# wangheda/youtube-8m

Measured on AMD Instinct MI355X. Metric: training videos/sec, higher is better.
Workload: dtype f32; 1 GPU; BASELINE configs[3]: LstmModel (2 x BasicLSTMCell(1024), dynamic_rnn over F=300) on raw uint8 [B,300,1152] frames + MoeModel head (2 mixtures, V=4716), fp32 training step (fwd+bwd+clip+Adam); per_gpu_batch=128, global_batch=128, frames=300, parallelism=dp1, params=113902808

## Files before the change

### include/yt8m_hip.h

```cpp
#ifndef YT8M_HIP_H
#define YT8M_HIP_H
#include <stdint.h>

#ifdef __cplusplus
extern "C" {
#endif

typedef void* yt8m_stream_t;

enum yt8m_status { YT8M_OK = 0, YT8M_E_BADARG = -1, YT8M_E_SHAPE = -2, YT8M_E_HIP = -3, YT8M_E_RCCL = -4 };
enum yt8m_label_dtype { YT8M_LABEL_U8 = 0, YT8M_LABEL_F32 = 1 };

int yt8m_abi_version(void);
const char* yt8m_last_error(void);
const char* yt8m_built_arch(void);

int yt8m_prof_enable(int on);
int yt8m_prof_reset(void);
int yt8m_prof_get(int family, int64_t* launches, double* total_ms);
int yt8m_prof_get_flops(int family, double* flops);
int yt8m_prof_get_bytes(int family, double* bytes);

int yt8m_probe_mfma_f32(int iters, int blocks, float* sink, yt8m_stream_t stream);
int yt8m_probe_mfma_bf16(int iters, int blocks, int random_operands, float* sink, yt8m_stream_t stream);
int yt8m_probe_copy_f32(const float* src, float* dst, int64_t n, yt8m_stream_t stream);
int yt8m_probe_placement(int* out, int blocks, int spin_ticks, yt8m_stream_t stream);
int yt8m_stream_create_cu_mask(const uint32_t* mask, int words, yt8m_stream_t* stream);
int yt8m_stream_destroy(yt8m_stream_t stream);

int yt8m_gemm_f32(int transA, int transB, int64_t M, int64_t N, int64_t K,
                  const float* A, int64_t lda, const float* B, int64_t ldb,
                  float* C, int64_t ldc, const float* bias, float beta, yt8m_stream_t stream);

int yt8m_gemm_f32_batched(int transA, int transB, int64_t M, int64_t N, int64_t K,
                          const float* A, int64_t lda, int64_t strideA, const float* B, int64_t ldb, int64_t strideB,
                          float* C, int64_t ldc, int64_t strideC, float beta, int64_t batch, yt8m_stream_t stream);

typedef struct yt8m_gemm_problem {
  int64_t M, N, K;
  const void* A; int64_t lda;
  const void* B; int64_t ldb;
  float* C; int64_t ldc;
  const float* bias;
  float beta;
} yt8m_gemm_problem;
int64_t yt8m_gemm_workspace_bytes(void);
int yt8m_gemm_f32_grouped(int transA, int transB, int nprob, const yt8m_gemm_problem* probs, void* workspace,
                          int64_t workspace_bytes, yt8m_stream_t stream);
int yt8m_gemm_bf16_nt_grouped(int nprob, const yt8m_gemm_problem* probs, void* workspace, int64_t workspace_bytes,
                              yt8m_stream_t stream);
int64_t yt8m_x3_image_bytes(int64_t rows, int64_t K);
int yt8m_x3_split(const float* src, int64_t R, int64_t C, int64_t ld, float scale, void* plain, void* trans, yt8m_stream_t stream);
int yt8m_gemm_x3_nt_grouped(int nprob, const yt8m_gemm_problem* probs, void* workspace, int64_t workspace_bytes,
                            yt8m_stream_t stream);
int yt8m_h2_split(const float* src, int64_t R, int64_t C, int64_t ld, float scale, const float* dscale, void* plain, void* trans,
                  float* colpart, yt8m_stream_t stream);
int yt8m_h2_absmax(const float* src, int64_t R, int64_t C, int64_t ld, void* word, yt8m_stream_t stream);
int yt8m_h2_degraded(uint64_t* counts, int reset, yt8m_stream_t stream);
int yt8m_h2_split_dropout(const float* src, int64_t R, int64_t C, float scale, const float* dscale, void* plain, void* trans,
                          float keep_prob, uint64_t seed, int64_t offset, yt8m_stream_t stream);
int yt8m_h2_split_rowmax(const float* src, int64_t R, int64_t C, int64_t ld, const void* rowmax, float* inv, void* plain,
                         yt8m_stream_t stream);
int yt8m_h2_split_ex(const float* src, int64_t R, int64_t C, int64_t ld, float scale, const void* dscale, const float* rowscale, void* plain,
                     void* trans, void* trans_scaled, float* colpart, float* colpart_scaled, yt8m_stream_t stream);
int yt8m_gemm_h1x2_nt_ex(int64_t M, int64_t N, int64_t K, const void* A1, int64_t ska, const void* B2, int64_t skb, float* C, int64_t ldc,
                         const float* bias, float alpha, const void* dsb, const float* rowscale, const float* colsum, float colsum_scale,
                         float beta, void* workspace, int64_t workspace_bytes, yt8m_stream_t stream);
int yt8m_h2_rowscales(const float* src, int64_t R, int64_t C, int64_t ld, float* S, float* inv, yt8m_stream_t stream);
int yt8m_h2_split_rows(const float* src, int64_t R, int64_t C, int64_t ld, const float* S, void* plain, yt8m_stream_t stream);
int yt8m_gemm_h2_nt_ex(int64_t M, int64_t N, int64_t K, const void* A2, int64_t ska, const void* B2, int64_t skb, float* C, int64_t ldc,
                       const float* bias, float alpha, const void* dsa, const void* dsb, const float* rowscale, float beta, void* workspace,
                       int64_t workspace_bytes, yt8m_stream_t stream);
int yt8m_timepool_max_f32(const float* y, int64_t F, int64_t B, int64_t N, int64_t ldy, float* out, int32_t* idx, int64_t ldo,
                          yt8m_stream_t stream);
int yt8m_timepool_shiftmax_f32(const float* z, int64_t F, int64_t B, int64_t ldz, int nfilt, const int32_t* fs, const int32_t* ncol, float* out,
                               int32_t* idx, int64_t ldo, yt8m_stream_t stream);
int yt8m_u8_cnn_pool_dw(const uint8_t* q, const float* r_tm, const int32_t* idx, const float* g, int64_t ldg, int64_t B, int64_t F, int64_t D,
                        int64_t N, int64_t fs, float* dW, float beta, yt8m_stream_t stream);
int yt8m_f32_cnn_pool_dw(const float* x, int64_t ldx, const int32_t* idx, const float* g, int64_t ldg, int64_t B, int64_t F, int64_t D,
                         int64_t N, int64_t fs, float* dW, int64_t lddw, float beta, yt8m_stream_t stream);
int yt8m_f32_cnn_pool_dx(const int32_t* idx, const float* g, int64_t ldg, int64_t B, int64_t F, int64_t D, int nfilt, const float* const* wt,
                         const int32_t* fs, const int32_t* ncol, float* dx, int64_t lddx, yt8m_stream_t stream);
int yt8m_u8_frames_image_f16(const uint8_t* q, const int32_t* num_frames, int64_t B, int64_t F, int64_t D, float eps, void* image,
                             float* x_tm, float* r_out, yt8m_stream_t stream);
int yt8m_u8_frames_image_t_f16(const uint8_t* q, const int32_t* num_frames, int64_t B, int64_t F, int64_t D, void* image_t,
                               yt8m_stream_t stream);
int yt8m_gemm_h2_nt_grouped(int nprob, const yt8m_gemm_problem* probs, const float* alphas, const float* const* dsa,
                            const float* const* dsb, void* workspace, int64_t workspace_bytes, yt8m_stream_t stream);
int yt8m_x3_set_combine(int mode);
int yt8m_x3_set_schedule(int mode);
#define YT8M_GEMM_ROLE_DW 0x100
#define YT8M_GEMM_ROLE_H2 0x200
int yt8m_gemm_x3_pays(int64_t M, int64_t N, int64_t K);
int64_t yt8m_gemm_auto_scratch_bytes(int transA, int transB, int nprob, const yt8m_gemm_problem* probs);
int yt8m_gemm_auto_grouped(int transA, int transB, int nprob, const yt8m_gemm_problem* probs, void* workspace,
                           int64_t workspace_bytes, void* image_scratch, int64_t image_scratch_bytes, uint64_t* used_x3,
                           yt8m_stream_t stream);
int yt8m_gemm_auto_grouped_ex(int transA, int transB, int nprob, const yt8m_gemm_problem* probs, const float* const* absmaxA,
                              const float* const* absmaxB, void* workspace, int64_t workspace_bytes, void* image_scratch,
                              int64_t image_scratch_bytes, uint64_t* used_x3, yt8m_stream_t stream);
int yt8m_gemm_x1x3_nt(int64_t M, int64_t N, int64_t K, const void* A1, const void* B3, float* C, int64_t ldc, const float* bias,
                      const float* rowscale, const float* colsum, float colsum_scale, void* workspace, int64_t workspace_bytes,
                      yt8m_stream_t stream);
int yt8m_gemm_x1x3_nt_ex(int64_t M, int64_t N, int64_t K, const void* A1, int64_t ska, const void* B3, int64_t skb, float* C,
                         int64_t ldc, const float* bias, float alpha, const float* rowscale, const float* colsum,
                         float colsum_scale, float beta, void* workspace, int64_t workspace_bytes, yt8m_stream_t stream);
int yt8m_bf16_image(const float* src, int64_t R, int64_t C, int64_t ld, float scale, void* plain, void* trans, yt8m_stream_t stream);
int yt8m_gemm_b1_nt_grouped(int nprob, const yt8m_gemm_problem* probs, void* workspace, int64_t workspace_bytes, yt8m_stream_t stream);
int yt8m_gemm_b1_nt_grouped_bf16c(int nprob, const yt8m_gemm_problem* probs, unsigned c_bf16_mask, void* workspace, int64_t workspace_bytes,
                                  yt8m_stream_t stream);
int yt8m_moe_mix_fwd_bf16z(const void* Zg, const void* Ze, float* p, int64_t B, int64_t V, int M, yt8m_stream_t stream);
int yt8m_moe_mix_bwd_bf16_images_z16(const void* Zg, const void* Ze, const float* dp, const void* labels, int label_dtype, int64_t B,
                                     int64_t V, int M, float eps, float dscale, const float* upstream_dev, void* dZg_img, int64_t g_kb,
                                     void* dZg_t_img, int64_t gt_kb, void* dZe_img, int64_t e_kb, void* dZe_t_img, int64_t et_kb,
                                     float* be_part, yt8m_stream_t stream);
int yt8m_bf16_image_colsum(const float* src, int64_t R, int64_t C, int64_t ld, float scale, const float* rowscale, void* plain,
                           void* trans, void* trans_scaled, float* colpart, float* colpart_scaled, yt8m_stream_t stream);
int yt8m_gemm_b1_nt_ex(int64_t M, int64_t N, int64_t K, const void* A1, int64_t ska, const void* B1, int64_t skb, float* C, int64_t ldc,
                       const float* bias, float alpha, const float* rowscale, const float* colsum, float colsum_scale, float beta,
                       void* workspace, int64_t workspace_bytes, yt8m_stream_t stream);
int yt8m_x3_split_ex(const float* src, int64_t R, int64_t C, int64_t ld, float scale, const float* rowscale, void* plain,
                     void* trans, void* trans_scaled, yt8m_stream_t stream);
int yt8m_x3_split_colsum(const float* src, int64_t R, int64_t C, int64_t ld, float scale, const float* rowscale, void* plain,
                         void* trans, void* trans_scaled, float* colpart, float* colpart_scaled, yt8m_stream_t stream);
int yt8m_cast_f32_bf16(const float* src, int64_t rows, int64_t cols, int64_t ld, void* dst, int64_t dst_ld, int transpose,
                       yt8m_stream_t stream);
int yt8m_cast_f32_bf16_dual(const float* src, int64_t rows, int64_t cols, int64_t ld, void* dst_plain, int64_t plain_ld,
                            void* dst_trans, int64_t trans_ld, yt8m_stream_t stream);

int yt8m_l2norm_fwd_f32(const float* x, float* y, int64_t rows, int64_t cols, float eps, yt8m_stream_t stream);
int yt8m_l2norm_bwd_f32(const float* x, const float* dy, float* dx, int64_t rows, int64_t cols, float eps,
                        yt8m_stream_t stream);
int yt8m_dequant_l2norm_u8(const uint8_t* q, const int32_t* num_frames, float* x,
                           int64_t B, int64_t F, int64_t D, float eps, yt8m_stream_t stream);
int yt8m_dequant_mean_l2norm_u8(const uint8_t* q, const int32_t* num_frames, float* x,
                                int64_t B, int64_t F, int64_t D, float eps, yt8m_stream_t stream);
int yt8m_resolution_mean_u8(const uint8_t* q, const int32_t* num_frames, float* y, int32_t* num_frames_out, int64_t B, int64_t F,
// ... 590 lines not shown
```

### youtube-8m_amd/csrc/common.h

```cpp
#pragma once
#include <hip/hip_runtime.h>
#include <stdint.h>
#include <stdio.h>
#include <string.h>
#include "../../include/yt8m_hip.h"

namespace yt8m {

extern thread_local char g_err[512];

inline int fail(int code, const char* fmt, const char* a = "", long long b = 0, long long c = 0) {
  snprintf(g_err, sizeof(g_err), fmt, a, b, c);
  return code;
}

#define YT8M_HIP_CHECK(expr)                                                              \
  do {                                                                                    \
    hipError_t _e = (expr);                                                               \
    if (_e != hipSuccess) {                                                               \
      snprintf(yt8m::g_err, sizeof(yt8m::g_err), "%s failed: %s (%s:%d)", #expr,          \
               hipGetErrorString(_e), __FILE__, __LINE__);                                \
      return YT8M_E_HIP;                                                                  \
    }                                                                                     \
  } while (0)

#define YT8M_REQUIRE(cond, code, msg)                                                     \
  do {                                                                                    \
    if (!(cond)) {                                                                        \
      snprintf(yt8m::g_err, sizeof(yt8m::g_err), "%s: requirement failed: %s", __func__, msg); \
      return code;                                                                        \
    }                                                                                     \
  } while (0)

enum Family { F_GEMM = 0, F_MOE_FUSED = 1, F_ELEMENTWISE = 2, F_OPTIM = 3, F_LSTM = 4, F_NETVLAD = 5, F_LSTM_BWD = 6, F_GEMM_X3 = 7,
              F_GEMM_X1X3 = 8,
              F_VLAD_ROWS = 9,
              F_VLAD_COLS = 10,
              F_NETVLAD_FWD = 11,
              F_GEMM_H2 = 12,
              F_GEMM_H1X2 = 13,
              F_COUNT = 14 };

struct ProfScope {
  int fam;
  hipStream_t s;
  bool on;
  hipEvent_t e0, e1;
  double flops;
  double bytes;
  ProfScope(int family, hipStream_t stream, double algorithmic_flops = 0.0, double algorithmic_bytes = 0.0);
  ~ProfScope();
};

bool prof_enabled();

struct GraphKey {
  int kind;
  int pad;
  const void* p[10];
  int64_t v[8];
};
}
#include <atomic>
#include <functional>
namespace yt8m {
int run_chain(const GraphKey& key, hipStream_t s, const std::function<int()>& launch_all);

inline hipStream_t as_stream(yt8m_stream_t s) { return reinterpret_cast<hipStream_t>(s); }

bool gemm_bf16_big_ok(int nprob, const yt8m_gemm_problem* probs);
int gemm_bf16_big_launch(int nprob, const yt8m_gemm_problem* probs, void* workspace, int64_t workspace_bytes, hipStream_t s);

struct DeviceOnce {
  std::atomic<bool> done[64];
  DeviceOnce() { for (auto& d : done) d.store(false); }
  hipError_t lds(const void* fn, int bytes) {
    int dev = 0;
    hipError_t e = hipGetDevice(&dev);
    if (e != hipSuccess) return e;
    if (dev >= 0 && dev < 64 && done[dev].load(std::memory_order_acquire)) return hipSuccess;
    e = hipFuncSetAttribute(fn, hipFuncAttributeMaxDynamicSharedMemorySize, bytes);
    if (e == hipSuccess && dev >= 0 && dev < 64) done[dev].store(true, std::memory_order_release);
    return e;
  }
};

inline int launch_status(const char* what) {
  hipError_t e = hipGetLastError();
  if (e != hipSuccess) {
    snprintf(g_err, sizeof(g_err), "launch of %s failed: %s", what, hipGetErrorString(e));
    return YT8M_E_HIP;
  }
  return YT8M_OK;
}

}

inline bool aligned16(const void* p) { return (reinterpret_cast<uintptr_t>(p) & 15) == 0; }
inline int64_t cdiv(int64_t a, int64_t b) { return (a + b - 1) / b; }
inline int64_t up4(int64_t a) { return (a + 3) & ~(int64_t)3; }

__device__ __forceinline__ float wave_sum(float v) {
#pragma unroll
  for (int o = 32; o > 0; o >>= 1) v += __shfl_xor(v, o, 64);
  return v;
}
__device__ __forceinline__ float wave_max(float v) {
#pragma unroll
  for (int o = 32; o > 0; o >>= 1) v = fmaxf(v, __shfl_xor(v, o, 64));
  return v;
}
__device__ __forceinline__ float block_sum_256(float v, float* red ) {
  v = wave_sum(v);
  const int lane = threadIdx.x & 63, w = threadIdx.x >> 6;
  __syncthreads();
  if (lane == 0) red[w] = v;
  __syncthreads();
  return red[0] + red[1] + red[2] + red[3];
}
__device__ __forceinline__ float block_max_256(float v, float* red) {
  v = wave_max(v);
  const int lane = threadIdx.x & 63, w = threadIdx.x >> 6;
  __syncthreads();
  if (lane == 0) red[w] = v;
  __syncthreads();
  return fmaxf(fmaxf(red[0], red[1]), fmaxf(red[2], red[3]));
}
template <int N>
__device__ __forceinline__ void block_sums_256(float (&v)[N], float* red ) {
#pragma unroll
  for (int k = 0; k < N; ++k) v[k] = wave_sum(v[k]);
  const int lane = threadIdx.x & 63, w = threadIdx.x >> 6;
  __syncthreads();
  if (lane == 0) {
#pragma unroll
    for (int k = 0; k < N; ++k) red[w * N + k] = v[k];
  }
  __syncthreads();
#pragma unroll
  for (int k = 0; k < N; ++k) v[k] = red[k] + red[N + k] + red[2 * N + k] + red[3 * N + k];
}
__device__ __forceinline__ float sigmoidf_(float z) { return 1.0f / (1.0f + expf(-z)); }

__device__ __forceinline__ float fast_sigmoid(float x) {
  return __builtin_amdgcn_rcpf(1.0f + __builtin_amdgcn_exp2f(-1.4426950408889634f * x));
}
__device__ __forceinline__ float fast_tanh(float x) {
  return 1.0f - 2.0f * __builtin_amdgcn_rcpf(1.0f + __builtin_amdgcn_exp2f(2.8853900817779268f * x));
}

template <int VW>
__device__ __forceinline__ void ldv(const float* p, float (&r)[VW]) {
  if constexpr (VW == 4) {
    const float4 q = *reinterpret_cast<const float4*>(p);
// ... 22 lines not shown
```

### youtube-8m_amd/csrc/gemm_f32.hip

```cpp
#include "common.h"

#ifdef YT8M_GEMM_TIMING
__device__ unsigned long long yt8m_gemm_phase[8];
extern "C" int yt8m_debug_gemm_phase(unsigned long long* out) {
  return hipMemcpyFromSymbol(out, HIP_SYMBOL(yt8m_gemm_phase), sizeof(unsigned long long) * 8) == hipSuccess ? 0 : -3;
}
#endif

#ifndef YT8M_GEMM_TEPI
#define YT8M_GEMM_TEPI 0
#endif

namespace {

constexpr bool TEPI = YT8M_GEMM_TEPI != 0;
constexpr int BM = 128, BN = 128, BK = 16;
constexpr int TILE_FLOATS = BK * 128;
constexpr int STAGES = 3;

typedef float f32x16 __attribute__((ext_vector_type(16)));

struct GemmArgs {
  const float* A;
  const float* B;
// ... 594 lines not shown

static int grouped_launch(int transA, int transB, int bf16, int nprob, const yt8m_gemm_problem* probs, void* workspace,
                          int64_t workspace_bytes, yt8m_stream_t stream) {
  using namespace yt8m;
  YT8M_REQUIRE(nprob >= 1 && nprob <= MAX_GROUP && probs, YT8M_E_BADARG, "1..4 problems");
  GroupArgs G;
  G.nprob = 0;
  int64_t T = 0;
  for (int i = 0; i < nprob; ++i) {
    const yt8m_gemm_problem& q = probs[i];
    GemmArgs g;
    int rc;
    if (bf16) {
      YT8M_REQUIRE(q.K % 2 == 0 && q.lda % 2 == 0 && q.ldb % 2 == 0, YT8M_E_SHAPE, "bf16 GEMM needs even K / lda / ldb");
      rc = fill_problem(g, 0, 1, q.M, q.N, q.K / 2, static_cast<const float*>(q.A), q.lda / 2, static_cast<const float*>(q.B),
                        q.ldb / 2, q.C, q.ldc, q.bias, q.beta);
    } else {
      rc = fill_problem(g, transA, transB, q.M, q.N, q.K, static_cast<const float*>(q.A), q.lda, static_cast<const float*>(q.B),
                        q.ldb, q.C, q.ldc, q.bias, q.beta);
    }
    if (rc != YT8M_OK) return rc;
    if (q.M == 0 || q.N == 0) continue;
    G.p[G.nprob] = g;
    G.tile_base[G.nprob] = (int)T;
    T += (int64_t)g.tiles_m * g.tiles_n;
    ++G.nprob;
  }
  if (G.nprob == 0) return YT8M_OK;
  YT8M_REQUIRE(T < (1LL << 30), YT8M_E_SHAPE, "too many tiles");
  for (int i = G.nprob; i <= MAX_GROUP; ++i) G.tile_base[i] = (int)T;
  for (int i = G.nprob; i < MAX_GROUP; ++i) G.p[i] = G.p[0];
  G.T = (int)T;
  G.P = T < SLOTS ? (int)T : SLOTS;
  G.full_rounds = (int)(T / G.P);
  G.rem = (int)(T - (int64_t)G.full_rounds * G.P);
  G.S = 1;
  G.ws = static_cast<float*>(workspace);
  if (T < SLOTS) {
    G.P = SLOTS;
    G.full_rounds = 0;
    G.rem = (int)T;
  }
  if (G.rem > 0) {
    int min_nk = 1 << 30, max_nk = 0;
    for (int i = 0; i < G.nprob; ++i) {
      const int nk = (G.p[i].K + BK - 1) / BK;
      if (nk < min_nk) min_nk = nk;
      if (nk > max_nk) max_nk = nk;
    }
    int Smax = min_nk / 8;
    if (Smax > 96) Smax = 96;
    const int64_t ws_items = workspace ? workspace_bytes / ((int64_t)BM * BN * (int64_t)sizeof(float)) : 0;
    if ((int64_t)G.rem * Smax > ws_items) Smax = (int)(ws_items / G.rem);
    int S = 1;
    double best = 1e30;
    for (int c = 1; c <= Smax; ++c) {
      const int64_t rounds = ((int64_t)G.rem * c + G.P - 1) / G.P;
      const double cost = (double)rounds * ((double)max_nk / c + 8.0) + (c > 1 ? 2.0 : 0.0);
      if (cost < best * 0.98) { best = cost; S = c; }
    }
    G.S = S;
  }
  hipStream_t s = as_stream(stream);
  double fl = 0.0;
  for (int i = 0; i < G.nprob; ++i) fl += 2.0 * (double)G.p[i].M * (double)G.p[i].N * (double)G.p[i].K;
  ProfScope prof(F_GEMM, s, fl);
  const int64_t grid = (int64_t)G.full_rounds * G.P + (int64_t)G.rem * G.S;
  int kmax = 0;
  for (int i = 0; i < G.nprob; ++i) kmax = std::max(kmax, G.p[i].K);
  if (bf16)
    hipLaunchKernelGGL((gemm_grouped_kernel<true, true, true>), dim3((unsigned)grid), dim3(256), 0, s, G);
  else if (transA && !transB && kmax <= 2048)
    hipLaunchKernelGGL((gemm_grouped_kernel<false, false, false, true>), dim3((unsigned)grid), dim3(256), 0, s, G);
  else
    launch_by_layout<GroupArgs>(transA, transB, gemm_grouped_kernel<true, false, false>, gemm_grouped_kernel<false, false, false>,
                                gemm_grouped_kernel<true, true, false>, gemm_grouped_kernel<false, true, false>,
                                dim3((unsigned)grid), s, G);
  if (G.S > 1) hipLaunchKernelGGL(splitk_fixup_kernel, dim3((unsigned)G.rem * 16), dim3(256), 0, s, G);
  return launch_status("gemm_grouped_kernel");
}

extern "C" int yt8m_gemm_f32_grouped(int transA, int transB, int nprob, const yt8m_gemm_problem* probs, void* workspace,
                                     int64_t workspace_bytes, yt8m_stream_t stream) {
  return grouped_launch(transA, transB, 0, nprob, probs, workspace, workspace_bytes, stream);
}

extern "C" int yt8m_gemm_bf16_nt_grouped(int nprob, const yt8m_gemm_problem* probs, void* workspace, int64_t workspace_bytes,
                                         yt8m_stream_t stream) {
  using namespace yt8m;
  YT8M_REQUIRE(nprob >= 1 && nprob <= MAX_GROUP && probs, YT8M_E_BADARG, "1..4 problems");
  bool simple = true;
  for (int i = 0; i < nprob; ++i) {
    const yt8m_gemm_problem& q = probs[i];
    simple = simple && q.M >= 0 && q.N >= 0 && q.K >= 0 && q.A && q.B && q.C && q.lda >= q.K && q.ldb >= q.K && q.ldc >= q.N &&
             (q.beta == 0.f || q.beta == 1.f);
  }
  if (simple && gemm_bf16_big_ok(nprob, probs)) {
    double fl = 0.0;
    for (int i = 0; i < nprob; ++i) fl += 2.0 * (double)probs[i].M * (double)probs[i].N * (double)probs[i].K;
    ProfScope prof(F_GEMM, as_stream(stream), fl);
    return gemm_bf16_big_launch(nprob, probs, workspace, workspace_bytes, as_stream(stream));
  }
  return grouped_launch(0, 1, 1, nprob, probs, workspace, workspace_bytes, stream);
}

extern "C" int yt8m_gemm_f32(int transA, int transB, int64_t M, int64_t N, int64_t K, const float* A, int64_t lda,
                             const float* B, int64_t ldb, float* C, int64_t ldc, const float* bias, float beta,
                             yt8m_stream_t stream) {
  return gemm_launch(transA, transB, M, N, K, A, lda, 0, B, ldb, 0, C, ldc, 0, bias, beta, 1, stream);
}

extern "C" int yt8m_gemm_f32_batched(int transA, int transB, int64_t M, int64_t N, int64_t K, const float* A, int64_t lda,
                                     int64_t strideA, const float* B, int64_t ldb, int64_t strideB, float* C, int64_t ldc,
                                     int64_t strideC, float beta, int64_t batch, yt8m_stream_t stream) {
  return gemm_launch(transA, transB, M, N, K, A, lda, strideA, B, ldb, strideB, C, ldc, strideC, nullptr, beta, batch, stream);
}
```

Baseline: 8316 videos/s.

## Route small-row fp32 GEMMs with large weights to bf16x3 MFMA row kernels

Adds a specialised path for fp32 GEMMs with at most 128 rows and large weight matrices, such as the MoE logits and the matching dx GEMMs. The activations are split into a three-term bf16 image. The weights are split on the fly into LDS, and a six-product bf16 MFMA sum emulates fp32 precision. The dx path uses split-K partials plus a combine kernel. The aim is to use matrix cores on these skinny, weight-bandwidth-bound GEMMs instead of the generic fp32 tiled kernel, at the cost of extra split launches, workspace use and small numeric differences.

```diff
diff --git a/include/yt8m_hip.h b/include/yt8m_hip.h
--- a/include/yt8m_hip.h
+++ b/include/yt8m_hip.h
@@ -53,6 +53,7 @@
 int yt8m_x3_split(const float* src, int64_t R, int64_t C, int64_t ld, float scale, void* plain, void* trans, yt8m_stream_t stream);
 int yt8m_gemm_x3_nt_grouped(int nprob, const yt8m_gemm_problem* probs, void* workspace, int64_t workspace_bytes,
                             yt8m_stream_t stream);
+#define YT8M_GEMM_ROLE_ROWS 0x400
 int yt8m_h2_split(const float* src, int64_t R, int64_t C, int64_t ld, float scale, const float* dscale, void* plain, void* trans,
                   float* colpart, yt8m_stream_t stream);
 int yt8m_h2_absmax(const float* src, int64_t R, int64_t C, int64_t ld, void* word, yt8m_stream_t stream);
diff --git a/youtube-8m_amd/csrc/common.h b/youtube-8m_amd/csrc/common.h
--- a/youtube-8m_amd/csrc/common.h
+++ b/youtube-8m_amd/csrc/common.h
@@ -70,6 +70,9 @@
 
 bool gemm_bf16_big_ok(int nprob, const yt8m_gemm_problem* probs);
 int gemm_bf16_big_launch(int nprob, const yt8m_gemm_problem* probs, void* workspace, int64_t workspace_bytes, hipStream_t s);
+bool gemm_rows_route(int transA, int transB, int nprob, const yt8m_gemm_problem* probs, int64_t workspace_bytes);
+int gemm_rows_logits(int nprob, const yt8m_gemm_problem* probs, void* workspace, int64_t workspace_bytes, yt8m_stream_t stream);
+int gemm_rows_dx(int nprob, const yt8m_gemm_problem* probs, void* workspace, int64_t workspace_bytes, yt8m_stream_t stream);
 
 struct DeviceOnce {
   std::atomic<bool> done[64];
diff --git a/youtube-8m_amd/csrc/gemm_f32.hip b/youtube-8m_amd/csrc/gemm_f32.hip
--- a/youtube-8m_amd/csrc/gemm_f32.hip
+++ b/youtube-8m_amd/csrc/gemm_f32.hip
@@ -700,6 +700,17 @@
 
 extern "C" int yt8m_gemm_f32_grouped(int transA, int transB, int nprob, const yt8m_gemm_problem* probs, void* workspace,
                                      int64_t workspace_bytes, yt8m_stream_t stream) {
+  const bool declared = (transA & YT8M_GEMM_ROLE_ROWS) != 0;
+  transA &= ~YT8M_GEMM_ROLE_ROWS;
+  if (declared) YT8M_REQUIRE(transA == 0 && nprob >= 1 && nprob <= MAX_GROUP && probs, YT8M_E_BADARG, "YT8M_GEMM_ROLE_ROWS: transA = 0, 1..4 problems");
+  if (declared || yt8m::gemm_rows_route(transA, transB, nprob, probs, workspace ? workspace_bytes : 0)) {
+    if (!transB) return yt8m::gemm_rows_logits(nprob, probs, workspace, workspace_bytes, stream);
+    for (int i = 0; i < nprob; ++i) {
+      const int rc = yt8m::gemm_rows_dx(1, probs + i, workspace, workspace_bytes, stream);
+      if (rc != YT8M_OK) return rc;
+    }
+    return YT8M_OK;
+  }
   return grouped_launch(transA, transB, 0, nprob, probs, workspace, workspace_bytes, stream);
 }
 
diff --git a/youtube-8m_amd/csrc/gemm_rows.hip b/youtube-8m_amd/csrc/gemm_rows.hip
--- /dev/null
+++ b/youtube-8m_amd/csrc/gemm_rows.hip
@@ -0,0 +1,518 @@
+#include "common.h"
+#include "rows_plan.h"
+#include <stdlib.h>
+
+namespace {
+
+using namespace yt8m_rows;
+
+typedef float f32x16 __attribute__((ext_vector_type(16)));
+typedef float f32x2 __attribute__((ext_vector_type(2)));
+typedef __bf16 bf16x8 __attribute__((ext_vector_type(8)));
+typedef __bf16 bf16x2 __attribute__((ext_vector_type(2)));
+typedef short s16x4 __attribute__((ext_vector_type(4)));
+typedef short s16x8 __attribute__((ext_vector_type(8)));
+
+constexpr int IMG_BLOCK_F = 256;
+
+__device__ __forceinline__ unsigned pk_bf16(float a, float b) {
+  const f32x2 f = {a, b};
+  return __builtin_bit_cast(unsigned, __builtin_convertvector(f, bf16x2));
+}
+__device__ __forceinline__ void split3_pair(float a, float b, unsigned& h0, unsigned& h1, unsigned& h2) {
+  h0 = pk_bf16(a, b);
+  const bool fa = (__float_as_uint(a) & 0x7F800000u) != 0x7F800000u, fb = (__float_as_uint(b) & 0x7F800000u) != 0x7F800000u;
+  const float ra = fa ? a - __uint_as_float(h0 << 16) : 0.f;
+  const float rb = fb ? b - __uint_as_float(h0 & 0xFFFF0000u) : 0.f;
+  h1 = pk_bf16(ra, rb);
+  h2 = pk_bf16(ra - __uint_as_float(h1 << 16), rb - __uint_as_float(h1 & 0xFFFF0000u));
+}
+__device__ __forceinline__ void store_split4(char* at, int plane, float4 v) {
+  unsigned a0, a1, a2, b0, b1, b2;
+  split3_pair(v.x, v.y, a0, a1, a2);
+  split3_pair(v.z, v.w, b0, b1, b2);
+  *reinterpret_cast<uint2*>(at) = make_uint2(a0, b0);
+  *reinterpret_cast<uint2*>(at + plane) = make_uint2(a1, b1);
+  *reinterpret_cast<uint2*>(at + 2 * plane) = make_uint2(a2, b2);
+}
+template <bool VEC>
+__device__ __forceinline__ float4 load4(const float* __restrict__ p, int c, int ncols, int ld, bool ok) {
+  float4 v = {0.f, 0.f, 0.f, 0.f};
+  if constexpr (VEC) {
+    v = *reinterpret_cast<const float4*>(p + min(c, ld - 4));
+  } else if (ok) {
+    if (c + 0 < ncols) v.x = p[c + 0];
+    if (c + 1 < ncols) v.y = p[c + 1];
+    if (c + 2 < ncols) v.z = p[c + 2];
+    if (c + 3 < ncols) v.w = p[c + 3];
+  }
+  return v;
+}
+__device__ __forceinline__ float4 mask4(float4 t, int c, int ncols, bool ok) {
+  float4 v;
+  v.x = (ok && c + 0 < ncols) ? t.x : 0.f;
+  v.y = (ok && c + 1 < ncols) ? t.y : 0.f;
+  v.z = (ok && c + 2 < ncols) ? t.z : 0.f;
+  v.w = (ok && c + 3 < ncols) ? t.w : 0.f;
+  return v;
+}
+__device__ __forceinline__ bf16x8 load_a(const float* __restrict__ img, int rg, int kb, int KB, int p, int li, int lk) {
+  const int64_t block = (int64_t)rg * KB + min(kb, KB - 1);
+  return __builtin_bit_cast(bf16x8, *reinterpret_cast<const float4*>(img + (block * 3 + p) * IMG_BLOCK_F + li * 8 + 4 * (lk ^ ((li >> 3) & 1))));
+}
+__device__ __forceinline__ bf16x8 keep_a(bf16x8 a, bool inside) {
+  return inside ? a : __builtin_bit_cast(bf16x8, make_float4(0.f, 0.f, 0.f, 0.f));
+}
+__device__ __forceinline__ f32x16 six(const bf16x8 (&a)[3], const bf16x8 (&b)[3], f32x16 c) {
+  c = __builtin_amdgcn_mfma_f32_32x32x16_bf16(a[2], b[0], c, 0, 0, 0);
+  c = __builtin_amdgcn_mfma_f32_32x32x16_bf16(a[1], b[0], c, 0, 0, 0);
+  c = __builtin_amdgcn_mfma_f32_32x32x16_bf16(a[1], b[1], c, 0, 0, 0);
+  c = __builtin_amdgcn_mfma_f32_32x32x16_bf16(a[0], b[0], c, 0, 0, 0);
+  c = __builtin_amdgcn_mfma_f32_32x32x16_bf16(a[0], b[1], c, 0, 0, 0);
+  c = __builtin_amdgcn_mfma_f32_32x32x16_bf16(a[0], b[2], c, 0, 0, 0);
+  return c;
+}
+constexpr int FLUSH_KBLOCKS = 8;
+template <int T>
+__device__ __forceinline__ void flush(f32x16 (&run)[T], f32x16 (&total)[T]) {
+#pragma unroll
+  for (int j = 0; j < T; ++j) {
+    total[j] += run[j];
+#pragma unroll
+    for (int r = 0; r < 16; ++r) run[j][r] = 0.f;
+  }
+}
+
+struct LArgs {
+  const float* W;
+  const float* img;
+  float* C;
+  const float* bias;
+  int64_t ldw, ldc;
+  int M, N, K, accumulate;
+};
+struct LGroup {
+  LArgs p[MAX_PROBS];
+  int slab_base[MAX_PROBS + 1];
+  int nprob;
+};
+
+constexpr int L_ROW_B = LOGITS_SLAB * 2;
+constexpr int L_PLANE_B = LOGITS_KBLK * L_ROW_B;
+constexpr int L_STAGE_B = 3 * L_PLANE_B;
+constexpr int L_LDS_B = 2 * L_STAGE_B;
+constexpr int L_LOADS = LOGITS_KBLK * (LOGITS_SLAB / 4) / 512;
+static_assert(LOGITS_KBLK * (LOGITS_SLAB / 4) % 512 == 0, "a stage is a whole number of float4 per thread");
+
+template <bool VEC>
+__global__ __launch_bounds__(512) void rows_logits_kernel(const LGroup G) {
+  extern __shared__ __attribute__((aligned(16))) char lds[];
+  int q = 0;
+  while (q + 1 < G.nprob && (int)blockIdx.x >= G.slab_base[q + 1]) ++q;
+  const LArgs& g = G.p[q];
+  const int n0 = ((int)blockIdx.x - G.slab_base[q]) * LOGITS_SLAB;
+  const int tid = threadIdx.x, lane = tid & 63, wave = tid >> 6;
+  const int li = lane & 31, lk = lane >> 5;
+  const int mt = wave & 3, kg = wave >> 2;
+  const int mtiles = (g.M + 31) >> 5;
+  const bool active = mt < mtiles;
+  const int rg = min(mt, mtiles - 1);
+  const int KB = (g.K + 15) >> 4;
+  const int nblk = (g.K + LOGITS_KBLK - 1) / LOGITS_KBLK;
+
+  int lrow[L_LOADS], lc4[L_LOADS];
+#pragma unroll
+  for (int i = 0; i < L_LOADS; ++i) {
+    const int idx = tid + 512 * i;
+    lrow[i] = idx / (LOGITS_SLAB / 4);
+    lc4[i] = idx % (LOGITS_SLAB / 4);
+  }
+  auto load_w = [&](int blk, float4 (&v)[L_LOADS]) __attribute__((always_inline)) {
+#pragma unroll
+    for (int i = 0; i < L_LOADS; ++i) {
+      const int k = blk * LOGITS_KBLK + lrow[i];
+      v[i] = load4<VEC>(g.W + (int64_t)min(k, g.K - 1) * g.ldw, n0 + lc4[i] * 4, g.N, (int)g.ldw, k < g.K);
+    }
+  };
+  auto store_w = [&](int blk, const float4 (&v)[L_LOADS]) __attribute__((always_inline)) {
+#pragma unroll
+    for (int i = 0; i < L_LOADS; ++i)
+      store_split4(lds + (blk & 1) * L_STAGE_B + lrow[i] * L_ROW_B + lc4[i] * 8, L_PLANE_B,
+                   mask4(v[i], n0 + lc4[i] * 4, g.N, blk * LOGITS_KBLK + lrow[i] < g.K));
+  };
+  auto keep_x = [&](int blk, const bf16x8 (&from)[2][3], bf16x8 (&to)[2][3]) __attribute__((always_inline)) {
+#pragma unroll
+    for (int s = 0; s < 2; ++s)
+#pragma unroll
+      for (int p = 0; p < 3; ++p) to[s][p] = keep_a(from[s][p], blk * (LOGITS_KBLK / 16) + 2 * kg + s < KB);
+  };
+  auto load_x = [&](int blk, bf16x8 (&a)[2][3]) __attribute__((always_inline)) {
+#pragma unroll
+    for (int s = 0; s < 2; ++s) {
+      const int kb = blk * (LOGITS_KBLK / 16) + 2 * kg + s;
+#pragma unroll
+      for (int p = 0; p < 3; ++p) a[s][p] = load_a(g.img, rg, kb, KB, p, li, lk);
+    }
+  };
+  const int tq = (lane >> 2) & 3, tp = lane & 3, gq = lane >> 4;
+  const int tr_off = (8 * (gq >> 1) + tq) * L_ROW_B + (16 * (gq & 1) + 4 * tp) * 2;
+
+  f32x16 acc[3], run[3];
+#pragma unroll
+  for (int j = 0; j < 3; ++j)
+#pragma unroll
+    for (int r = 0; r < 16; ++r) acc[j][r] = run[j][r] = 0.f;
+
+  float4 wv[L_LOADS];
+  bf16x8 xa[2][3], xn[2][3];
+  load_w(0, wv);
+  load_x(0, xn);
+  store_w(0, wv);
+  keep_x(0, xn, xa);
+  __syncthreads();
+  for (int blk = 0; blk < nblk; ++blk) {
+    const bool more = blk + 1 < nblk;
+    const int nxt = more ? blk + 1 : blk;
+    load_w(nxt, wv);
+    load_x(nxt, xn);
+    __builtin_amdgcn_sched_barrier(0);
+    {
+      const char* S = lds + (blk & 1) * L_STAGE_B + tr_off;
+#pragma unroll
+      for (int s = 0; s < 2; ++s) {
+        const char* Sk = S + (2 * kg + s) * 16 * L_ROW_B;
+#pragma unroll
+        for (int j = 0; j < 3; ++j) {
+          bf16x8 b[3];
+#pragma unroll
+          for (int p = 0; p < 3; ++p) {
+            const char* at = Sk + p * L_PLANE_B + j * 64;
+            const s16x4 lo = __builtin_amdgcn_ds_read_tr16_b64_v4i16((__attribute__((address_space(3))) s16x4*)(at));
+            const s16x4 hi = __builtin_amdgcn_ds_read_tr16_b64_v4i16((__attribute__((address_space(3))) s16x4*)(at + 4 * L_ROW_B));
+            const s16x8 both = {lo[0], lo[1], lo[2], lo[3], hi[0], hi[1], hi[2], hi[3]};
+            b[p] = __builtin_bit_cast(bf16x8, both);
+          }
+          run[j] = six(xa[s], b, run[j]);
+        }
+      }
+    }
+    if ((blk + 1) % (FLUSH_KBLOCKS / 2) == 0) flush(run, acc);
+    __builtin_amdgcn_sched_barrier(0);
+    if (more) {
+      store_w(blk + 1, wv);
+      keep_x(blk + 1, xn, xa);
+    }
+    __syncthreads();
+  }
+  flush(run, acc);
+  float* X = reinterpret_cast<float*>(lds) + (mt * 3 * 16) * 64 + lane;
+  if (kg == 1) {
+#pragma unroll
+    for (int j = 0; j < 3; ++j)
+#pragma unroll
+      for (int r = 0; r < 16; ++r) X[(j * 16 + r) * 64] = acc[j][r];
+  }
+  __syncthreads();
+  if (kg == 1 || !active) return;
+#pragma unroll
+  for (int j = 0; j < 3; ++j) {
+    const int col = n0 + 32 * j + li;
+    if (col >= g.N) continue;
+    const float bv = g.bias ? g.bias[col] : 0.f;
+#pragma unroll
+    for (int r = 0; r < 16; ++r) {
+      const int row = mt * 32 + (r & 3) + 8 * (r >> 2) + 4 * lk;
+      if (row < g.M) {
+        float* c = g.C + (int64_t)row * g.ldc + col;
+        float v = acc[j][r] + X[(j * 16 + r) * 64] + bv;
+        if (g.accumulate) v += *c;
+        *c = v;
+      }
+    }
+  }
+}
+
+struct DArgs {
+  const float* W[MAX_PROBS];
+  const float* img[MAX_PROBS];
+  int64_t ldw[MAX_PROBS];
+  int N[MAX_PROBS];
+  int split_prob[DX_MAX_SPLITS], split_g0[DX_MAX_SPLITS], split_g1[DX_MAX_SPLITS];
+  float* part;
+  float* C;
+  int64_t ldc;
+  int M, Kout, S, accumulate;
+};
+
+constexpr int D_ROW_B = DX_GROUP * 2 + 16;
+constexpr int D_PLANE_B = DX_SLAB * D_ROW_B;
+constexpr int D_STAGE_B = 3 * D_PLANE_B;
+constexpr int D_LDS_B = 2 * D_STAGE_B;
+constexpr int D_LOADS = DX_SLAB * (DX_GROUP / 4) / 512;
+
+template <bool VEC>
+__global__ __launch_bounds__(512) void rows_dx_kernel(const DArgs g) {
+  extern __shared__ __attribute__((aligned(16))) char lds[];
+  const int split = (int)blockIdx.x % g.S, slab = (int)blockIdx.x / g.S;
+  const int q = g.split_prob[split], g0 = g.split_g0[split], g1 = g.split_g1[split];
+  const int tid = threadIdx.x, lane = tid & 63, wave = tid >> 6;
+  const int li = lane & 31, lk = lane >> 5;
+  const int mt = wave & 3, cp = wave >> 2;
+  const int mtiles = (g.M + 31) >> 5;
+  const bool active = mt < mtiles;
+  const int rg = min(mt, mtiles - 1);
+  const int N = g.N[q];
+  const int KB = (N + 15) >> 4;
+  const int64_t ldw = g.ldw[q];
+  const int o0 = slab * DX_SLAB;
+  const float* W = g.W[q];
+  const float* img = g.img[q];
+
+  int lrow[D_LOADS], lc4[D_LOADS];
+#pragma unroll
+  for (int i = 0; i < D_LOADS; ++i) {
+    const int idx = tid + 512 * i;
+    lrow[i] = idx / (DX_GROUP / 4);
+    lc4[i] = idx % (DX_GROUP / 4);
+  }
+  auto load_w = [&](int grp, float4 (&v)[D_LOADS]) __attribute__((always_inline)) {
+#pragma unroll
+    for (int i = 0; i < D_LOADS; ++i) {
+      const int row = o0 + lrow[i];
+      v[i] = load4<VEC>(W + (int64_t)min(row, g.Kout - 1) * ldw, grp * DX_GROUP + lc4[i] * 4, N, (int)ldw, row < g.Kout);
+    }
+  };
+  auto store_w = [&](int grp, const float4 (&v)[D_LOADS]) __attribute__((always_inline)) {
+#pragma unroll
+    for (int i = 0; i < D_LOADS; ++i)
+      store_split4(lds + ((grp - g0) & 1) * D_STAGE_B + lrow[i] * D_ROW_B + lc4[i] * 8, D_PLANE_B,
+                   mask4(v[i], grp * DX_GROUP + lc4[i] * 4, N, o0 + lrow[i] < g.Kout));
+  };
+  auto keep_z = [&](int grp, const bf16x8 (&from)[4][3], bf16x8 (&to)[4][3]) __attribute__((always_inline)) {
+#pragma unroll
+    for (int s = 0; s < 4; ++s)
+#pragma unroll
+      for (int p = 0; p < 3; ++p) to[s][p] = keep_a(from[s][p], grp * (DX_GROUP / 16) + s < KB);
+  };
+  auto load_z = [&](int grp, int s, bf16x8 (&a)[3]) __attribute__((always_inline)) {
+    const int kb = grp * (DX_GROUP / 16) + s;
+#pragma unroll
+    for (int p = 0; p < 3; ++p) a[p] = load_a(img, rg, kb, KB, p, li, lk);
+  };
+
+  f32x16 acc[2], run[2];
+#pragma unroll
+  for (int j = 0; j < 2; ++j)
+#pragma unroll
+    for (int r = 0; r < 16; ++r) acc[j][r] = run[j][r] = 0.f;
+
+  float4 wv[D_LOADS];
+  bf16x8 za[4][3], zn[4][3];
+  load_w(g0, wv);
+#pragma unroll
+  for (int s = 0; s < 4; ++s) load_z(g0, s, zn[s]);
+  store_w(g0, wv);
+  keep_z(g0, zn, za);
+  __syncthreads();
+  for (int grp = g0; grp < g1; ++grp) {
+    const int st = (grp - g0) & 1;
+    const bool more = grp + 1 < g1;
+    const int nxt = more ? grp + 1 : grp;
+    load_w(nxt, wv);
+#pragma unroll
+    for (int s = 0; s < 4; ++s) load_z(nxt, s, zn[s]);
+    __builtin_amdgcn_sched_barrier(0);
+    {
+      const char* S = lds + st * D_STAGE_B + (64 * cp + li) * D_ROW_B + lk * 16;
+#pragma unroll
+      for (int s = 0; s < 4; ++s) {
+#pragma unroll
+        for (int j = 0; j < 2; ++j) {
+          bf16x8 b[3];
+#pragma unroll
+          for (int p = 0; p < 3; ++p)
+            b[p] = __builtin_bit_cast(bf16x8, *reinterpret_cast<const float4*>(S + p * D_PLANE_B + j * 32 * D_ROW_B + s * 32));
+          run[j] = six(za[s], b, run[j]);
+        }
+      }
+    }
+    if ((grp - g0 + 1) % (FLUSH_KBLOCKS / 4) == 0) flush(run, acc);
+    __builtin_amdgcn_sched_barrier(0);
+    if (more) {
+      store_w(grp + 1, wv);
+      keep_z(grp + 1, zn, za);
+    }
+    __syncthreads();
+  }
+  flush(run, acc);
+  if (!active) return;
+  float* P = g.part + ((int64_t)slab * g.S + split) * (MAX_ROWS * DX_SLAB);
+#pragma unroll
+  for (int j = 0; j < 2; ++j)
+#pragma unroll
+    for (int r = 0; r < 16; ++r) {
+      const int row = mt * 32 + (r & 3) + 8 * (r >> 2) + 4 * lk;
+      P[row * DX_SLAB + 64 * cp + 32 * j + li] = acc[j][r];
+    }
+}
+
+__global__ __launch_bounds__(256) void rows_dx_combine_kernel(const float* __restrict__ part, float* __restrict__ C, int64_t ldc, int M,
+                                                              int Kout, int S, int accumulate) {
+  const int o4 = (Kout + 3) >> 2;
+  const int64_t idx = (int64_t)blockIdx.x * 256 + threadIdx.x;
+  if (idx >= (int64_t)M * o4) return;
+  const int m = (int)(idx / o4), o = (int)(idx % o4) * 4;
+  const int slab = o / DX_SLAB, c = o % DX_SLAB;
+  const float* p = part + (int64_t)slab * S * (MAX_ROWS * DX_SLAB) + m * DX_SLAB + c;
+  float4 v = *reinterpret_cast<const float4*>(p);
+  for (int s = 1; s < S; ++s) {
+    const float4 t = *reinterpret_cast<const float4*>(p + (int64_t)s * (MAX_ROWS * DX_SLAB));
+    v.x += t.x; v.y += t.y; v.z += t.z; v.w += t.w;
+  }
+  float* c4 = C + (int64_t)m * ldc + o;
+  if (o + 3 < Kout && (ldc & 3) == 0 && (reinterpret_cast<uintptr_t>(C) & 15) == 0) {
+    if (accumulate) {
+      const float4 old = *reinterpret_cast<const float4*>(c4);
+      v.x += old.x; v.y += old.y; v.z += old.z; v.w += old.w;
+    }
+    *reinterpret_cast<float4*>(c4) = v;
+  } else {
+    const float vv[4] = {v.x, v.y, v.z, v.w};
+    for (int e = 0; e < 4 && o + e < Kout; ++e) c4[e] = accumulate ? vv[e] + c4[e] : vv[e];
+  }
+}
+
+}
+
+using namespace yt8m;
+
+static bool rows_enabled() {
+  static const bool off = getenv("YT8M_GEMM_ROWS") != nullptr && atoi(getenv("YT8M_GEMM_ROWS")) == 0;
+  return !off;
+}
+
+static int64_t rows_workspace_bytes(bool dx, int nprob, const yt8m_gemm_problem* probs) {
+  int64_t M[MAX_PROBS], N[MAX_PROBS], K[MAX_PROBS];
+  int same[MAX_PROBS];
+  for (int i = 0; i < nprob; ++i) {
+    M[i] = probs[i].M; N[i] = probs[i].N; K[i] = probs[i].K;
+    same[i] = i;
+    for (int j = 0; j < i; ++j)
+      if (probs[j].A == probs[i].A && probs[j].lda == probs[i].lda && M[j] == M[i] && K[j] == K[i]) { same[i] = j; break; }
+  }
+  if (dx) return plan_dx(nprob, M[0], N[0], K).workspace_bytes;
+  return plan_logits(nprob, M, N, K, same).workspace_bytes;
+}
+
+bool yt8m::gemm_rows_route(int transA, int transB, int nprob, const yt8m_gemm_problem* probs, int64_t workspace_bytes) {
+  if (!rows_enabled() || transA != 0 || nprob < 1 || nprob > MAX_PROBS || !probs) return false;
+  if (transB && nprob != 1) return false;
+  for (int i = 0; i < nprob; ++i) {
+    const yt8m_gemm_problem& q = probs[i];
+    if (!(q.beta == 0.f || q.beta == 1.f) || !q.A || !q.B || !q.C) return false;
+    if (transB ? !route(q.M, q.N, q.K, q.ldb) : !route(q.M, q.K, q.N, q.ldb)) return false;
+    if (transB && q.bias) return false;
+  }
+  return rows_workspace_bytes(transB != 0, nprob, probs) <= workspace_bytes;
+}
+
+int yt8m::gemm_rows_logits(int nprob, const yt8m_gemm_problem* probs, void* workspace, int64_t workspace_bytes, yt8m_stream_t stream) {
+  YT8M_REQUIRE(nprob >= 1 && nprob <= MAX_PROBS && probs, YT8M_E_BADARG, "1..4 problems");
+  int64_t M[MAX_PROBS], N[MAX_PROBS], K[MAX_PROBS];
+  int same[MAX_PROBS];
+  for (int i = 0; i < nprob; ++i) {
+    const yt8m_gemm_problem& q = probs[i];
+    YT8M_REQUIRE(supported(q.M, q.K, q.N, q.ldb) && q.lda >= q.K && q.ldc >= q.N, YT8M_E_SHAPE, "1..128 rows, ld >= width");
+    YT8M_REQUIRE(q.A && q.B && q.C && (q.beta == 0.f || q.beta == 1.f), YT8M_E_BADARG, "operands and beta in {0, 1}");
+    M[i] = q.M; N[i] = q.N; K[i] = q.K;
+    same[i] = i;
+    for (int j = 0; j < i; ++j)
+      if (probs[j].A == q.A && probs[j].lda == q.lda && M[j] == M[i] && K[j] == K[i]) { same[i] = j; break; }
+  }
+  const LogitsPlan pl = plan_logits(nprob, M, N, K, same);
+  YT8M_REQUIRE(workspace && workspace_bytes >= pl.workspace_bytes && (reinterpret_cast<uintptr_t>(workspace) & 15) == 0, YT8M_E_BADARG,
+               "workspace too small (yt8m_gemm_workspace_bytes) or unaligned");
+  LGroup G;
+  G.nprob = nprob;
+  for (int i = 0; i <= MAX_PROBS; ++i) G.slab_base[i] = pl.slab_base[std::min(i, nprob)];
+  for (int i = 0; i < MAX_PROBS; ++i) {
+    const int s = std::min(i, nprob - 1);
+    const yt8m_gemm_problem& q = probs[s];
+    void* img = static_cast<char*>(workspace) + pl.image_off[s];
+    if (i < nprob && same[i] == i) {
+      int rc = yt8m_x3_split(static_cast<const float*>(q.A), q.M, q.K, q.lda, 1.0f, img, nullptr, stream);
+      if (rc != YT8M_OK) return rc;
+    }
+    G.p[i] = LArgs{static_cast<const float*>(q.B), static_cast<const float*>(img), q.C, q.bias, q.ldb, q.ldc, (int)q.M, (int)q.N,
+                   (int)q.K, q.beta != 0.f ? 1 : 0};
+  }
+  bool vec = true;
+  for (int i = 0; i < nprob; ++i) vec = vec && (probs[i].ldb & 3) == 0 && aligned16(probs[i].B);
+  static DeviceOnce once_v, once_s;
+  YT8M_HIP_CHECK(vec ? once_v.lds(reinterpret_cast<const void*>(rows_logits_kernel<true>), L_LDS_B)
+                     : once_s.lds(reinterpret_cast<const void*>(rows_logits_kernel<false>), L_LDS_B));
+  hipStream_t s = as_stream(stream);
+  double fl = 0.0;
+  for (int i = 0; i < nprob; ++i) fl += 2.0 * (double)M[i] * (double)N[i] * (double)K[i];
+  ProfScope prof(F_GEMM_X3, s, fl);
+  if (vec) hipLaunchKernelGGL(rows_logits_kernel<true>, dim3((unsigned)pl.grid()), dim3(512), L_LDS_B, s, G);
+  else hipLaunchKernelGGL(rows_logits_kernel<false>, dim3((unsigned)pl.grid()), dim3(512), L_LDS_B, s, G);
+  return launch_status("rows_logits_kernel");
+}
+
+int yt8m::gemm_rows_dx(int nprob, const yt8m_gemm_problem* probs, void* workspace, int64_t workspace_bytes, yt8m_stream_t stream) {
+  YT8M_REQUIRE(nprob >= 1 && nprob <= MAX_PROBS && probs, YT8M_E_BADARG, "1..4 problems");
+  const int64_t M = probs[0].M, Kout = probs[0].N;
+  int64_t N[MAX_PROBS];
+  for (int i = 0; i < nprob; ++i) {
+    const yt8m_gemm_problem& q = probs[i];
+    YT8M_REQUIRE(q.M == M && q.N == Kout, YT8M_E_SHAPE, "the problems of a dx launch share rows and output columns");
+    YT8M_REQUIRE(supported(q.M, q.N, q.K, q.ldb) && q.lda >= q.K, YT8M_E_SHAPE, "1..128 rows, ld >= width");
+    YT8M_REQUIRE(q.A && q.B, YT8M_E_BADARG, "operands");
+    N[i] = q.K;
+  }
+  const yt8m_gemm_problem& q0 = probs[0];
+  YT8M_REQUIRE(q0.C && q0.ldc >= Kout && (q0.beta == 0.f || q0.beta == 1.f), YT8M_E_BADARG, "output and beta in {0, 1}");
+  const DxPlan pl = plan_dx(nprob, M, Kout, N);
+  YT8M_REQUIRE(workspace && workspace_bytes >= pl.workspace_bytes && (reinterpret_cast<uintptr_t>(workspace) & 15) == 0, YT8M_E_BADARG,
+               "workspace too small (yt8m_gemm_workspace_bytes) or unaligned");
+  DArgs g;
+  for (int i = 0; i < MAX_PROBS; ++i) {
+    const int s = std::min(i, nprob - 1);
+    const yt8m_gemm_problem& q = probs[s];
+    void* img = static_cast<char*>(workspace) + pl.image_off[s];
+    if (i < nprob) {
+      int rc = yt8m_x3_split(static_cast<const float*>(q.A), q.M, q.K, q.lda, 1.0f, img, nullptr, stream);
+      if (rc != YT8M_OK) return rc;
+    }
+    g.W[i] = static_cast<const float*>(q.B);
+    g.img[i] = static_cast<const float*>(img);
+    g.ldw[i] = q.ldb;
+    g.N[i] = (int)q.K;
+  }
+  for (int i = 0; i < DX_MAX_SPLITS; ++i) {
+    const int s = std::min(i, pl.S - 1);
+    g.split_prob[i] = pl.split_prob[s]; g.split_g0[i] = pl.split_g0[s]; g.split_g1[i] = pl.split_g1[s];
+  }
+  g.part = reinterpret_cast<float*>(static_cast<char*>(workspace) + pl.partial_off);
+  g.C = q0.C;
+  g.ldc = q0.ldc;
+  g.M = (int)M; g.Kout = (int)Kout; g.S = pl.S; g.accumulate = q0.beta != 0.f ? 1 : 0;
+  bool vec = true;
+  for (int i = 0; i < nprob; ++i) vec = vec && (probs[i].ldb & 3) == 0 && aligned16(g.W[i]);
+  static DeviceOnce once_v, once_s;
+  YT8M_HIP_CHECK(vec ? once_v.lds(reinterpret_cast<const void*>(rows_dx_kernel<true>), D_LDS_B)
+                     : once_s.lds(reinterpret_cast<const void*>(rows_dx_kernel<false>), D_LDS_B));
+  hipStream_t s = as_stream(stream);
+  double fl = 0.0;
+  for (int i = 0; i < nprob; ++i) fl += 2.0 * (double)M * (double)Kout * (double)N[i];
+  ProfScope prof(F_GEMM_X3, s, fl);
+  if (vec) hipLaunchKernelGGL(rows_dx_kernel<true>, dim3((unsigned)pl.grid()), dim3(512), D_LDS_B, s, g);
+  else hipLaunchKernelGGL(rows_dx_kernel<false>, dim3((unsigned)pl.grid()), dim3(512), D_LDS_B, s, g);
+  int rc = launch_status("rows_dx_kernel");
+  if (rc != YT8M_OK) return rc;
+  const int64_t threads = M * ((Kout + 3) / 4);
+  hipLaunchKernelGGL(rows_dx_combine_kernel, dim3((unsigned)::cdiv(threads, 256)), dim3(256), 0, s, g.part, g.C, g.ldc, g.M, g.Kout, g.S,
+                     g.accumulate);
+  return launch_status("rows_dx_combine_kernel");
+}
diff --git a/youtube-8m_amd/csrc/rows_plan.h b/youtube-8m_amd/csrc/rows_plan.h
--- /dev/null
+++ b/youtube-8m_amd/csrc/rows_plan.h
@@ -0,0 +1,99 @@
+#pragma once
+#include <algorithm>
+#include <cstdint>
+
+namespace yt8m_rows {
+
+constexpr int MAX_ROWS = 128;
+constexpr int MAX_PROBS = 4;
+constexpr int LOGITS_SLAB = 96;
+constexpr int LOGITS_KBLK = 64;
+constexpr int DX_SLAB = 128;
+constexpr int DX_GROUP = 64;
+constexpr int DX_MAX_SPLITS = 16;
+constexpr int TARGET_WGS = 256;
+constexpr int64_t MIN_WEIGHT_ELEMS = (int64_t)1 << 24;
+constexpr int64_t MIN_WEIGHT_DIM = 1024;
+
+inline int64_t cdiv(int64_t a, int64_t b) { return (a + b - 1) / b; }
+inline int64_t up256(int64_t v) { return (v + 255) / 256 * 256; }
+inline int64_t image_bytes(int64_t rows, int64_t K) { return cdiv(rows, 32) * cdiv(K, 16) * 3072; }
+
+inline bool route(int64_t M, int64_t wrows, int64_t wcols, int64_t ldw) {
+  return M >= 1 && M <= MAX_ROWS && ldw == wcols && wrows >= MIN_WEIGHT_DIM && wcols >= MIN_WEIGHT_DIM &&
+         wrows < ((int64_t)1 << 30) && wcols < ((int64_t)1 << 30) && wrows * wcols >= MIN_WEIGHT_ELEMS;
+}
+inline bool supported(int64_t M, int64_t wrows, int64_t wcols, int64_t ldw) {
+  return M >= 1 && M <= MAX_ROWS && wrows >= 1 && wcols >= 1 && ldw >= wcols && wrows < ((int64_t)1 << 30) &&
+         wcols < ((int64_t)1 << 30) && ldw < ((int64_t)1 << 31);
+}
+
+struct LogitsPlan {
+  int nprob = 0;
+  int slab_base[MAX_PROBS + 1] = {};
+  int64_t image_off[MAX_PROBS] = {};
+  int64_t workspace_bytes = 0;
+  int grid() const { return slab_base[nprob]; }
+};
+inline LogitsPlan plan_logits(int nprob, const int64_t* M, const int64_t* N, const int64_t* K, const int* same_a) {
+  LogitsPlan pl;
+  pl.nprob = nprob;
+  int64_t off = 0;
+  for (int p = 0; p < nprob; ++p) {
+    pl.slab_base[p + 1] = pl.slab_base[p] + (int)cdiv(N[p], LOGITS_SLAB);
+    if (same_a[p] != p) {
+      pl.image_off[p] = pl.image_off[same_a[p]];
+    } else {
+      pl.image_off[p] = off;
+      off += up256(image_bytes(M[p], K[p]));
+    }
+  }
+  pl.workspace_bytes = off;
+  return pl;
+}
+
+struct DxPlan {
+  int nprob = 0;
+  int slabs = 0;
+  int S = 0;
+  int split_prob[DX_MAX_SPLITS] = {};
+  int split_g0[DX_MAX_SPLITS] = {};
+  int split_g1[DX_MAX_SPLITS] = {};
+  int64_t image_off[MAX_PROBS] = {};
+  int64_t partial_off = 0;
+  int64_t workspace_bytes = 0;
+  int grid() const { return slabs * S; }
+};
+inline DxPlan plan_dx(int nprob, int64_t M, int64_t Kout, const int64_t* N) {
+  DxPlan pl;
+  pl.nprob = nprob;
+  pl.slabs = (int)cdiv(Kout, DX_SLAB);
+  int64_t groups[MAX_PROBS], total = 0;
+  for (int p = 0; p < nprob; ++p) { groups[p] = cdiv(N[p], DX_GROUP); total += groups[p]; }
+  int64_t want = std::max<int64_t>(1, (TARGET_WGS + pl.slabs / 2) / std::max(pl.slabs, 1));
+  want = std::min<int64_t>(std::min<int64_t>(want, DX_MAX_SPLITS), total);
+  want = std::max<int64_t>(want, nprob);
+  int sp[MAX_PROBS];
+  int64_t given = 0;
+  for (int p = 0; p < nprob; ++p) {
+    int64_t s = p + 1 < nprob ? (want * groups[p] + total / 2) / total : want - given;
+    s = std::max<int64_t>(1, std::min<int64_t>(s, std::min<int64_t>(groups[p], want - given - (nprob - 1 - p))));
+    sp[p] = (int)s;
+    given += s;
+  }
+  pl.S = (int)given;
+  int at = 0;
+  for (int p = 0; p < nprob; ++p)
+    for (int j = 0; j < sp[p]; ++j, ++at) {
+      pl.split_prob[at] = p;
+      pl.split_g0[at] = (int)(groups[p] * j / sp[p]);
+      pl.split_g1[at] = (int)(groups[p] * (j + 1) / sp[p]);
+    }
+  int64_t off = 0;
+  for (int p = 0; p < nprob; ++p) { pl.image_off[p] = off; off += up256(image_bytes(M, N[p])); }
+  pl.partial_off = off;
+  pl.workspace_bytes = off + (int64_t)pl.slabs * pl.S * MAX_ROWS * DX_SLAB * 4;
+  return pl;
+}
+
+}
```

Result: no change. 8355 videos/s, median of 6 (+0.5%).
